# bioinfologics/w2rap-contigger

Measured on AMD Instinct MI355X. Metric: step2_k60_canonical_kmers_per_s, higher is better.
Workload: dtype u64

## Files before the change

### include/w2rap_step2.h

```cpp
#ifndef W2RAP_STEP2_H_
#define W2RAP_STEP2_H_

#include <stddef.h>
#include <stdint.h>

#ifdef __cplusplus
extern "C" {
#endif

#define W2RAP_STEP2_ABI_VERSION 3

enum {
    W2RAP_OK = 0,
    W2RAP_E_ARG = 1,
    W2RAP_E_NO_DEVICE = 2,
    W2RAP_E_HIP = 3,
    W2RAP_E_STATE = 4,
    W2RAP_E_LIMIT = 5,
    W2RAP_E_GRAPH = 6,
    W2RAP_E_HINT = 7,
    W2RAP_E_IO = 8
};

enum { W2RAP_MEM_HOST = 0, W2RAP_MEM_DEVICE = 1 };
// ... 3 lines not shown
    const uint8_t*  bases_packed;
    const uint64_t* base_byte_off;
    const uint32_t* read_len;
    const uint8_t*  quals;
    const uint64_t* qual_off;
    const uint8_t*  pq;
    const uint64_t* pq_off;
    int32_t mem;
} w2rap_reads;

typedef struct w2rap_edge_hint {
    uint64_t n_edges;
    const uint8_t*  packed;
    const uint64_t* byte_off;
    const uint32_t* len;
} w2rap_edge_hint;

typedef struct w2rap_step2_params {
    uint32_t K;
    uint32_t min_qual;
    uint32_t min_freq;
    int32_t  device;
    const w2rap_edge_hint* edge_order_hint;
    const char* freqs_path;
    int32_t  n_gpus;
    uint32_t n_passes;
    const int32_t* devices;
    uint32_t flags;
} w2rap_step2_params;
#define W2RAP_F_REPLICATED_GRAPH 1u
#define W2RAP_F_GRAPH_ONLY 2u

typedef struct w2rap_step2_out {
    int32_t  K;
    uint64_t n_vertices;
    uint64_t n_edge_objs;
    uint8_t*  edge_packed;
    uint64_t* edge_byte_off;
    uint32_t* edge_len;
    int32_t*  vleft;
    int32_t*  vright;
    uint64_t* from_off;
    int32_t*  from_v;
    int32_t*  from_e;
    uint64_t* to_off;
    int32_t*  to_v;
    int32_t*  to_e;
    uint64_t n_unipaths;
    int32_t*  fwd_xlat;
    int32_t*  rev_xlat;
    uint64_t n_paths;
    int32_t*  path_offset;
    uint64_t* path_off;
    int32_t*  path_edges;
    uint64_t hist[101];
    uint64_t n_kmer_instances;
    uint64_t n_kmers_distinct;
    uint64_t n_kmers_solid;
    uint64_t n_reads_pathed;
    uint64_t n_reads_multipathed;
    float ms_count, ms_graph, ms_path;
} w2rap_step2_out;

int  w2rap_step2_run(const w2rap_reads* reads, const w2rap_step2_params* params,
                     w2rap_step2_out* out, char* err, size_t errlen);
void w2rap_step2_free(w2rap_step2_out* out);
int  w2rap_step2_device_count(void);
int  w2rap_step2_abi_version(void);
int  w2rap_step2_last_peer_mode(void);

int  w2rap_step2_trim_cached(void);
struct w2rap_step2_ctx* w2rap_step2_acquire(int device, char* err, size_t errlen);
void w2rap_step2_release(struct w2rap_step2_ctx*);

typedef struct w2rap_step2_ctx w2rap_step2_ctx;

w2rap_step2_ctx* w2rap_step2_create(int device, char* err, size_t errlen);
void        w2rap_step2_destroy(w2rap_step2_ctx*);
const char* w2rap_step2_last_error(const w2rap_step2_ctx*);
int w2rap_step2_set_reads(w2rap_step2_ctx*, const w2rap_reads* reads);
int w2rap_step2_count_kmers(w2rap_step2_ctx*, uint32_t min_qual, uint32_t min_freq, w2rap_step2_out* stats);
int w2rap_step2_count_kmers_passes(w2rap_step2_ctx*, uint32_t min_qual, uint32_t min_freq, uint32_t n_passes, w2rap_step2_out* stats);
int w2rap_step2_build_graph(w2rap_step2_ctx*, const w2rap_edge_hint* hint);
int w2rap_step2_path_reads(w2rap_step2_ctx*);
int w2rap_step2_fetch(w2rap_step2_ctx*, w2rap_step2_out* out);
void* w2rap_step2_stream(w2rap_step2_ctx*);

int w2rap_step2_trim(w2rap_step2_ctx*);

int w2rap_step2_copy_bench(w2rap_step2_ctx*, uint64_t nbytes, uint32_t reps, double* gb_per_s);
int w2rap_step2_device_copy(w2rap_step2_ctx*, void* dst, const void* src, uint64_t nbytes);
int w2rap_step2_copy_bench_form(void);

int    w2rap_step2_set_profiling(w2rap_step2_ctx*, int on);
size_t w2rap_step2_profile(w2rap_step2_ctx*, char* buf, size_t len, int reset);

int w2rap_step2_counts(w2rap_step2_ctx*, uint64_t out[8]);

int w2rap_step2_get_good_len(w2rap_step2_ctx*, uint16_t* out );
int w2rap_step2_get_table(w2rap_step2_ctx*, uint64_t* hi, uint64_t* lo, uint8_t* count, uint8_t* ctx,
                          int32_t* edge, uint32_t* off );

int      w2rap_step2_quality_windows(w2rap_step2_ctx*, uint32_t min_qual, uint64_t* n_kmers );
uint32_t w2rap_step2_default_buckets(uint64_t total_kmers, uint32_t multiple_of);
uint32_t w2rap_step2_record_bytes(void);
int w2rap_step2_partition(w2rap_step2_ctx*, uint32_t n_buckets, uint32_t n_parts, uint64_t* recs_per_part,
                          uint64_t* kmers_per_part);
int w2rap_step2_partition_range(w2rap_step2_ctx*, uint32_t n_buckets, uint32_t first_bucket, uint32_t end_bucket, uint32_t n_parts,
                                uint64_t* recs_per_part, uint64_t* kmers_per_part);
int w2rap_step2_count_pass(w2rap_step2_ctx*, uint32_t pass, uint32_t n_passes);
int w2rap_step2_partition_buffers(w2rap_step2_ctx*, void** d_records, void** d_bucket_counts, uint64_t* n_records);
int w2rap_step2_count_records(w2rap_step2_ctx*, uint32_t min_freq, uint32_t n_local_buckets, uint32_t n_segments,
                              const void* d_records, const void* d_counts, uint64_t total_kmers, w2rap_step2_out* stats);
int w2rap_step2_count_records_begin(w2rap_step2_ctx*, uint32_t min_freq, uint32_t n_local_buckets, uint32_t n_segments,
                                    const void* d_records, const void* d_counts, uint64_t total_kmers, uint32_t n_slices,
                                    int deferred);
int w2rap_step2_count_records_slices(w2rap_step2_ctx*);
int w2rap_step2_count_records_bounds(w2rap_step2_ctx*, uint32_t k, uint32_t* first_bucket, uint32_t* end_bucket);
int w2rap_step2_count_records_launch(w2rap_step2_ctx*, uint32_t k);
int w2rap_step2_count_records_slice(w2rap_step2_ctx*, uint32_t k, uint64_t* n_solid, uint64_t* n_chunks);
int w2rap_step2_count_records_end(w2rap_step2_ctx*, w2rap_step2_out* stats);
int w2rap_step2_solid_buffers(w2rap_step2_ctx*, void** d_hi, void** d_lo, void** d_cc, uint64_t* n);
int w2rap_step2_set_solid(w2rap_step2_ctx*, const void* d_hi, const void* d_lo, const void* d_cc, uint64_t n,
                          uint64_t M, uint64_t D, const uint64_t* hist101);
int w2rap_step2_chunk_buffers(w2rap_step2_ctx*, void** d_chunk_start, void** d_chunk_count, uint64_t* n_chunks);
int w2rap_step2_set_solid_chunked(w2rap_step2_ctx*, const void* d_hi, const void* d_lo, const void* d_cc, uint64_t n,
                                  uint64_t M, uint64_t D, const uint64_t* hist101,
                                  const void* d_chunk_start, const void* d_chunk_count, uint64_t n_chunks);

int w2rap_step2_dict_begin(w2rap_step2_ctx*, uint64_t kmer_capacity, uint64_t chunk_capacity);
int w2rap_step2_dict_append(w2rap_step2_ctx*, const void* d_hi, const void* d_lo, const void* d_cc, uint64_t n,
                            const void* d_chunk_start, const void* d_chunk_count, uint64_t n_chunks);
int w2rap_step2_dict_append_slice(w2rap_step2_ctx*, const void* d_hi, const void* d_lo, const void* d_cc, uint64_t n,
                                  const void* d_chunk_start, const void* d_chunk_count, uint64_t n_chunks, uint64_t chunk_bias);
int w2rap_step2_dict_end(w2rap_step2_ctx*, uint64_t M, uint64_t D, const uint64_t* hist101);
int w2rap_step2_dict_abort(w2rap_step2_ctx*);

enum { W2RAP_X_DONE = 0, W2RAP_X_ALLTOALL = 1, W2RAP_X_ALLGATHER = 2, W2RAP_X_ALLGATHER_HOST = 3, W2RAP_X_ALLREDUCE_U8 = 4, W2RAP_X_ALLREDUCE_U32 = 5 };
typedef struct w2rap_xchg {
    int32_t  op;
    uint32_t elem_bytes;
    void*    send;
    uint64_t send_count[64];
} w2rap_xchg;
int w2rap_step2_shard_begin(w2rap_step2_ctx*, uint32_t rank, uint32_t world, const uint64_t* solid_per_rank ,
                            uint32_t n_buckets, uint32_t n_passes, uint64_t M, uint64_t D, const uint64_t* hist101,
                            const w2rap_edge_hint* hint );
int w2rap_step2_local_dict_slice(w2rap_step2_ctx*, uint64_t n_solid, uint64_t expected_total);
int w2rap_step2_shard_next(w2rap_step2_ctx*, w2rap_xchg* x);
int w2rap_step2_shard_recv(w2rap_step2_ctx*, const uint64_t* recv_count , uint32_t elem_bytes, void** d_recv);
int w2rap_step2_shard_host_words(w2rap_step2_ctx*, const uint64_t* words );
int w2rap_step2_shard_info(w2rap_step2_ctx*, uint64_t out[8]);
int w2rap_step2_selftest_prims(w2rap_step2_ctx*, uint64_t n, uint64_t seed, int key_bits);
uint64_t w2rap_step2_device_bytes(w2rap_step2_ctx*);
uint64_t w2rap_step2_device_peak_bytes(w2rap_step2_ctx*, int reset);

#ifdef __cplusplus
}
#endif
#endif
```

### w2rap_contigger_amd/csrc/step2_graph.hip

```cpp
#include <algorithm>
#include "ctx.h"

namespace w2 {

enum { GE_LOOKUP = 1, GE_OFFSET = 2, GE_HINT_MISS = 4, GE_HINT_DUP = 8, GE_ASSIGN = 16, GE_HINT_LEN = 32 };

template <class Id>
__device__ inline Kmer oriented(const uint64_t* shi, const uint64_t* slo, Id v) {
    Kmer k{shi[v >> 1], slo[v >> 1]};
    return (v & 1) ? kmer_rc(k) : k;
}

template <class Id>
__global__ void __launch_bounds__(256) k_links(uint64_t S, const uint64_t* __restrict__ shi, const uint64_t* __restrict__ slo,
                                                const uint8_t* __restrict__ sctx, Id* nbr_nxt0) {
    constexpr Id NONE = NodeId<Id>::NONE, PAL = NodeId<Id>::PAL;
    uint64_t i = (uint64_t)blockIdx.x * blockDim.x + threadIdx.x;
    if (i >= S) return;
    Kmer k{shi[i], slo[i]};
    Id n0 = NONE, n1 = NONE;
    if (!kmer_is_pal(k)) {
        const Id s = nbr_nxt0[2 * i], p = nbr_nxt0[2 * i + 1];
        if (s < PAL) {
            unsigned cj = sctx[s >> 1]; if (s & 1) cj = brev8(cj);
// ... 1203 lines not shown
    if (getenv("W2RAP_TRACE")) fprintf(stderr, "[w2rap] list ranking: %d jump launches\n", rounds);
    c.release(spl); c.release(d_cnt);
    if (mid) W2_HIP(hipMemsetAsync(mid, 0, N, st));
    LAUNCH(c, "k_rank_finish", k_rank_finish<Id>, dim3(grid_for(S)), dim3(256), 0, S, w, own, nxt0, shi, slo, nxt, rnk, cyc, mid, d_flags);
    W2_HIP(hipStreamSynchronize(st));
    return 0;
}
int run_ranking(Ctx& c, uint64_t N, const uint32_t* nxt0, uint32_t* nxt, uint32_t* rnk, unsigned long long* w, uint8_t* cyc, uint8_t* mid,
                uint32_t* d_flags, const uint64_t* shi, const uint64_t* slo, bool use_chunks) {
    uint32_t* own = nullptr;
    W2_ALLOC(own, uint32_t, N);
    const int rc = run_ranking_t<uint32_t>(c, N, nxt0, nxt, rnk, w, own, cyc, mid, d_flags, shi, slo, use_chunks);
    c.release(own);
    return rc;
}

static int graph_error(Ctx& c, uint32_t f) {
    if (f & GE_LOOKUP) { c.err = "neighbour k-mer lookup failed (ForceAssert, BuildReadQGraph.cc:265)"; return W2RAP_E_GRAPH; }
    if (f & GE_OFFSET) { c.err = "unipath longer than 16,777,215 k-mers (ForceAssertLe, ReadPather.h:122)"; return W2RAP_E_GRAPH; }
    if (f & GE_ASSIGN) { c.err = "k-mer left without an edge (BuildReadQGraph.cc:303)"; return W2RAP_E_GRAPH; }
    if (f & GE_HINT_MISS) { c.err = "edge_order_hint: a hinted edge is not a unipath of this graph"; return W2RAP_E_HINT; }
    if (f & GE_HINT_DUP) { c.err = "edge_order_hint: an edge is listed twice"; return W2RAP_E_HINT; }
    if (f & GE_HINT_LEN) { c.err = "edge_order_hint: a hinted edge has the wrong length"; return W2RAP_E_HINT; }
    return 0;
}

template <class Id>
static int rank_resolve_t(Ctx& c, uint64_t N, Id* nxt0, unsigned long long* rankw, uint32_t* own, uint8_t* cyc, uint8_t* mid, uint32_t* d_flags,
                          const uint64_t* shi, const uint64_t* slo, bool with_mid, bool* had_circles = nullptr) {
    hipStream_t st = c.stream;
    const uint64_t S = N / 2;
    uint32_t h_flags[4] = {0, 0, 0, 0};
    W2_TRY(run_ranking_t<Id>(c, N, nxt0, (Id*)nullptr, (uint32_t*)nullptr, rankw, own, cyc, mid, d_flags, with_mid ? shi : nullptr, slo, true));
    W2_HIP(hipMemcpyAsync(h_flags, d_flags, 16, hipMemcpyDeviceToHost, st));
    W2_HIP(hipStreamSynchronize(st));
    W2_TRY(graph_error(c, h_flags[1]));
    if (had_circles) *had_circles = h_flags[2] != 0;
    if (h_flags[2]) {
        Id *nx, *mn, *nx2, *mn2;
        W2_ALLOC(nx, Id, N); W2_ALLOC(mn, Id, N); W2_ALLOC(nx2, Id, N); W2_ALLOC(mn2, Id, N);
        LAUNCH(c, "k_minjump_init", k_minjump_init<Id>, dim3(grid_for(S)), dim3(256), 0, S, nxt0, cyc, nx, mn);
        for (int round = 0; round < 33; ++round) {
            LAUNCH(c, "k_minjump", k_minjump<Id>, dim3(grid_for(S)), dim3(256), 0, S, shi, slo, nx, mn, nx2, mn2);
            std::swap(nx, nx2); std::swap(mn, mn2);
        }
        LAUNCH(c, "k_cycle_cut", k_cycle_cut<Id>, dim3(grid_for(S)), dim3(256), 0, S, cyc, mn, nxt0);
        W2_HIP(hipStreamSynchronize(st));
        c.release(nx); c.release(mn); c.release(nx2); c.release(mn2);
        W2_HIP(hipMemsetAsync(d_flags, 0, 32, st));
        W2_TRY(run_ranking_t<Id>(c, N, nxt0, (Id*)nullptr, (uint32_t*)nullptr, rankw, own, cyc, mid, d_flags, with_mid ? shi : nullptr, slo, true));
        W2_HIP(hipMemcpyAsync(h_flags, d_flags, 16, hipMemcpyDeviceToHost, st));
        W2_HIP(hipStreamSynchronize(st));
        if (h_flags[2]) { c.err = "failed to close circle (BuildReadQGraph.cc:141)"; return W2RAP_E_GRAPH; }
    }
    return 0;
}
int rank_resolve32(Ctx& c, uint64_t N, uint32_t* nxt0, unsigned long long* rankw, uint32_t* own, uint8_t* cyc, uint8_t* mid, uint32_t* d_flags,
                   const uint64_t* shi, const uint64_t* slo, bool* had_circles) {
    return rank_resolve_t<uint32_t>(c, N, nxt0, rankw, own, cyc, mid, d_flags, shi, slo, false, had_circles);
}
int rank_resolve64(Ctx& c, uint64_t N, uint64_t* nxt0, unsigned long long* rankw, uint32_t* own, uint8_t* cyc, uint8_t* mid, uint32_t* d_flags,
                   const uint64_t* shi, const uint64_t* slo, bool* had_circles) {
    return rank_resolve_t<uint64_t>(c, N, nxt0, rankw, own, cyc, mid, d_flags, shi, slo, false, had_circles);
}

int graph_finish(Ctx& c) {
    hipStream_t st = c.stream;
    const uint64_t E = c.E;
    uint32_t* d_flags = nullptr;
    W2_ALLOC(d_flags, uint32_t, 8);
    W2_HIP(hipMemsetAsync(d_flags, 0, 32, st));
    uint32_t h_flags[4] = {0, 0, 0, 0};
    if (!c.bits_ready) {
        const uint64_t nby = (c.edge_bases + 3) / 4;
        W2_ALLOC(c.d_edge_bits, uint8_t, nby + 16);
        W2_HIP(hipMemsetAsync(c.d_edge_bits + nby, 0, 16, st));
        if (nby) LAUNCH(c, "k_pack_codes", k_pack_codes, dim3(grid_for(nby)), dim3(256), 0, nby, c.edge_bases, c.d_edge_codes, c.d_edge_bits);
    }
    c.bits_ready = false;
    if (c.use_index && c.d_table) { c.release(c.d_table); c.d_table = nullptr; }
    if (c.use_index && !c.index_prebuilt) W2_TRY(build_index(c));
    c.index_prebuilt = false;
    if (c.filter_prebuilt) c.filter_prebuilt = false;
    else {
    if (c.d_filter32) { c.release(c.d_filter32); c.d_filter32 = nullptr; }
    c.f32words = 0;
    if (c.edge_bases >= FMER && c.stream2 && !getenv("W2RAP_NO_FILTER32") && c.edge_bases <= (1ull << 33)) {
        uint64_t fw = 1024;
        while (fw * 4 < c.edge_bases) fw <<= 1;
        W2_ALLOC(c.d_filter32, unsigned long long, fw);
        c.f32words = fw;
        hipEvent_t ev;
        W2_HIP(hipEventCreateWithFlags(&ev, hipEventDisableTiming));
        W2_HIP(hipEventRecord(ev, st));
        W2_HIP(hipStreamWaitEvent(c.stream2, ev, 0));
        (void)hipEventDestroy(ev);
        W2_HIP(hipMemsetAsync(c.d_filter32, 0, fw * 8, c.stream2));
        const uint64_t npos = c.edge_bases - (FMER - 1);
        LAUNCH_ON(c, c.stream2, "k_filter32", k_filter32, dim3(grid_for(npos)), dim3(256), 0, npos, c.d_edge_bits, c.d_filter32, (uint32_t)(fw - 1), 0u, (uint32_t)fw);
    }
    }
    uint32_t* d_nobj = nullptr; uint64_t* d_ooff = nullptr;
    W2_ALLOC(d_nobj, uint32_t, E); W2_ALLOC(d_ooff, uint64_t, E + 1);
    if (E) LAUNCH(c, "k_edge_nobj", k_edge_nobj, dim3(grid_for(E)), dim3(256), 0, E, c.d_edge_nk, c.d_edge_off, c.d_edge_codes, d_nobj);
    W2_TRY(exclusive_scan_u32_to_u64(c, d_nobj, d_ooff, E));
    W2_HIP(hipMemcpyAsync(&c.NO, d_ooff + E, 8, hipMemcpyDeviceToHost, st));
    W2_HIP(hipMemcpyAsync(h_flags, d_flags, 16, hipMemcpyDeviceToHost, st));
    W2_HIP(hipStreamSynchronize(st));
    W2_TRY(graph_error(c, h_flags[1]));
    const uint64_t NO = c.NO;
    if (NO >= (1ull << 31)) { c.err = "more than 2^31 edge objects"; return W2RAP_E_LIMIT; }
    W2_ALLOC(c.d_fwdX, int32_t, E); W2_ALLOC(c.d_revX, int32_t, E); W2_ALLOC(c.d_obj_edge, uint32_t, NO);
    W2_ALLOC(c.d_left, int32_t, NO); W2_ALLOC(c.d_right, int32_t, NO);
    if (E) LAUNCH(c, "k_edge_xlat", k_edge_xlat, dim3(grid_for(E)), dim3(256), 0, E, d_nobj, d_ooff, c.d_fwdX, c.d_revX, c.d_obj_edge);
    const uint64_t NE = 2 * NO;
    uint64_t *ehash, *ehi, *elo, *ktmp, *excl;
    uint32_t *eperm, *eflag;
    W2_ALLOC(ehash, uint64_t, NE); W2_ALLOC(ehi, uint64_t, NE); W2_ALLOC(elo, uint64_t, NE); W2_ALLOC(ktmp, uint64_t, NE);
    W2_ALLOC(excl, uint64_t, NE + 1); W2_ALLOC(eperm, uint32_t, NE); W2_ALLOC(eflag, uint32_t, NE);
    c.NV = 0;
    if (NE) {
        LAUNCH(c, "k_ends", k_ends, dim3(grid_for(NE)), dim3(256), 0, NO, c.d_obj_edge, c.d_edge_off, c.d_edge_nk, c.d_edge_codes, ehash, ehi, elo);
        bool by_bases = test_hook("W2RAP_TEST_ENDS_FULL_SORT");
        uint64_t nflag = 0;
        for (;;) {
            LAUNCH(c, "k_iota", k_iota, dim3(grid_for(NE)), dim3(256), 0, NE, eperm);
            if (by_bases) {
                LAUNCH(c, "k_gather_u64", k_gather_u64, dim3(grid_for(NE)), dim3(256), 0, NE, elo, eperm, ktmp);
                W2_TRY(sort_pairs_u64(c, ktmp, eperm, NE, 0, 58));
                LAUNCH(c, "k_gather_u64", k_gather_u64, dim3(grid_for(NE)), dim3(256), 0, NE, ehi, eperm, ktmp);
                W2_TRY(sort_pairs_u64(c, ktmp, eperm, NE, 0, 60));
            }
            LAUNCH(c, "k_gather_u64", k_gather_u64, dim3(grid_for(NE)), dim3(256), 0, NE, ehash, eperm, ktmp);
            W2_TRY(sort_pairs_u64(c, ktmp, eperm, NE, 0, 64));
            W2_HIP(hipMemsetAsync(d_flags + 3, 0, 4, st));
            LAUNCH(c, "k_end_flags", k_end_flags, dim3(grid_for(NE)), dim3(256), 0, NE, eperm, ehash, ehi, elo, eflag, d_flags + 3);
            W2_TRY(exclusive_scan_u32_to_u64(c, eflag, excl, NE));
            uint32_t shared_hash = 0;
            W2_HIP(hipMemcpyAsync(&nflag, excl + NE, 8, hipMemcpyDeviceToHost, st));
            W2_HIP(hipMemcpyAsync(&shared_hash, d_flags + 3, 4, hipMemcpyDeviceToHost, st));
            W2_HIP(hipStreamSynchronize(st));
            if (shared_hash && !by_bases) { by_bases = true; continue; }
            break;
        }
        c.NV = nflag + 1;
        LAUNCH(c, "k_end_vertices", k_end_vertices, dim3(grid_for(NE)), dim3(256), 0, NE, eperm, eflag, excl, c.d_left, c.d_right);
    }
    const uint64_t NV = c.NV;
    W2_ALLOC(c.d_from_off, uint64_t, NV + 1); W2_ALLOC(c.d_to_off, uint64_t, NV + 1);
    W2_ALLOC(c.d_from_v, int32_t, NO); W2_ALLOC(c.d_from_e, int32_t, NO);
    W2_ALLOC(c.d_to_v, int32_t, NO); W2_ALLOC(c.d_to_e, int32_t, NO);
    uint32_t* deg = nullptr; uint64_t* akeys = nullptr; uint32_t* avals = nullptr;
    W2_ALLOC(deg, uint32_t, NV); W2_ALLOC(akeys, uint64_t, NO); W2_ALLOC(avals, uint32_t, NO);
    for (int dir = 0; dir < 2; ++dir) {
        const int32_t* a = dir == 0 ? c.d_left : c.d_right;
        const int32_t* b = dir == 0 ? c.d_right : c.d_left;
        W2_HIP(hipMemsetAsync(deg, 0, (NV ? NV : 1) * 4, st));
        if (NO) {
            LAUNCH(c, "k_adj_keys", k_adj_keys, dim3(grid_for(NO)), dim3(256), 0, NO, a, b, akeys, avals, deg);
            W2_TRY(sort_pairs_u64(c, akeys, avals, NO, 0, 64));
            LAUNCH(c, "k_adj_out", k_adj_out, dim3(grid_for(NO)), dim3(256), 0, NO, avals, b, dir == 0 ? c.d_from_v : c.d_to_v,
                               dir == 0 ? c.d_from_e : c.d_to_e);
        }
        W2_TRY(exclusive_scan_u32_to_u64(c, deg, dir == 0 ? c.d_from_off : c.d_to_off, NV));
    }
    if (c.d_otab) { c.release(c.d_otab); c.d_otab = nullptr; }
    W2_ALLOC(c.d_otab, ObjRec, NO);
    if (NO) LAUNCH(c, "k_obj_table", k_obj_table, dim3(grid_for(NO)), dim3(256), 0, NO, c.d_obj_edge, c.d_edge_nk, c.d_edge_off, c.d_edge_codes,
                   c.d_right, c.d_from_off, c.d_from_e, c.d_otab);
    W2_HIP(hipStreamSynchronize(st));
    if (c.stream2) W2_HIP(hipStreamSynchronize(c.stream2));
    W2_HIP(hipGetLastError());
    for (void* p : {(void*)d_nobj, (void*)d_ooff, (void*)ehash, (void*)ehi, (void*)elo, (void*)ktmp, (void*)excl,
                    (void*)eperm, (void*)eflag, (void*)deg, (void*)akeys, (void*)avals, (void*)d_flags})
        c.release(p);
    c.graphed = true;
    return 0;
}

template <class Id>
static int phase_graph_t(Ctx& c, const w2rap_edge_hint* hint) {
    constexpr Id NONE = NodeId<Id>::NONE; (void)NONE;
    hipStream_t st = c.stream;
    const uint64_t S = c.S, N = 2 * S;
    const uint64_t mask = c.tcap - 1;
    uint32_t* d_flags = nullptr;
    W2_ALLOC(d_flags, uint32_t, 8);
    W2_HIP(hipMemsetAsync(d_flags, 0, 32, st));
    Id* nxt0 = reinterpret_cast<Id*>(c.d_nbr);
    unsigned long long* rankw = nullptr; uint32_t* own = nullptr;
    W2_ALLOC(rankw, unsigned long long, N); W2_ALLOC(own, uint32_t, N);
    uint8_t *cyc = nullptr, *mid = nullptr, *is_head = nullptr;
    W2_ALLOC(cyc, uint8_t, N); W2_ALLOC(mid, uint8_t, N);
    uint32_t h_flags[4] = {0, 0, 0, 0};
    if (S) {
        LAUNCH(c, "k_links", k_links<Id>, dim3(grid_for(S)), dim3(256), 0, S, c.d_shi, c.d_slo, c.d_sctx, nxt0);
        W2_TRY(rank_resolve_t<Id>(c, N, nxt0, rankw, own, cyc, mid, d_flags, c.d_shi, c.d_slo, true));
    }
    c.release(cyc); cyc = nullptr;
    unsigned long long* d_nheads = nullptr;
    W2_ALLOC(d_nheads, unsigned long long, 1);
    W2_HIP(hipMemsetAsync(d_nheads, 0, 8, st));
    const uint64_t head_cap = S ? c.rank_ends + 1 : 1;
    Id *head_v, *edge_head; uint32_t* perm;
    uint64_t *key_hi, *key_lo, *key_tmp;
    W2_ALLOC(is_head, uint8_t, N);
    W2_ALLOC(head_v, Id, head_cap); W2_ALLOC(key_hi, uint64_t, head_cap); W2_ALLOC(key_lo, uint64_t, head_cap);
    if (S) LAUNCH(c, "k_heads", k_heads<Id>, dim3((unsigned)((S + 256 * HEADS_PER - 1) / (256 * HEADS_PER))), dim3(256), 0, S, c.d_shi, c.d_slo, nxt0, own, rankw, mid, is_head,
                              head_v, key_hi, key_lo, d_nheads, head_cap, d_flags, hint == nullptr);
    W2_HIP(hipGetLastError());
    unsigned long long E = 0;
    W2_HIP(hipMemcpyAsync(&E, d_nheads, 8, hipMemcpyDeviceToHost, st));
    W2_HIP(hipMemcpyAsync(h_flags, d_flags, 16, hipMemcpyDeviceToHost, st));
    W2_HIP(hipStreamSynchronize(st));
    W2_TRY(graph_error(c, h_flags[1]));
    if (E > head_cap) { c.err = "more canonical heads than chain ends"; return W2RAP_E_GRAPH; }
    if (E >= (1ull << 31)) { c.err = "more than 2^31 unipaths (edge ids are int, paths/long/ReadPath.h)"; return W2RAP_E_LIMIT; }
    c.E = E;
    c.release(c.d_nbr); c.d_nbr = nullptr; nxt0 = nullptr;
    c.release(mid); mid = nullptr;
    W2_ALLOC(perm, uint32_t, E); W2_ALLOC(edge_head, Id, E);
    W2_ALLOC(key_tmp, uint64_t, E);
    W2_ALLOC(c.d_edge_nk, uint32_t, E);
    if (hint) {
        if (hint->n_edges != E) {
            c.err = "edge_order_hint has " + std::to_string(hint->n_edges) + " edges, the graph has " + std::to_string(E);
            return W2RAP_E_HINT;
        }
        std::vector<uint64_t> hh(E), hl(E);
        for (uint64_t e = 0; e < E; ++e) {
            if (hint->len[e] < K) { c.err = "edge_order_hint: edge shorter than K"; return W2RAP_E_HINT; }
            const uint8_t* p = hint->packed + hint->byte_off[e];
            uint64_t hi = 0, lo = 0;
            for (unsigned t = 0; t < 30; ++t) hi = (hi << 2) | ((p[t >> 2] >> (2 * (t & 3))) & 3);
            for (unsigned t = 30; t < 60; ++t) lo = (lo << 2) | ((p[t >> 2] >> (2 * (t & 3))) & 3);
            hh[e] = hi; hl[e] = lo;
        }
        uint32_t* d_hlen = nullptr;
        W2_ALLOC(d_hlen, uint32_t, E);
        W2_HIP(hipMemcpyAsync(key_hi, hh.data(), E * 8, hipMemcpyHostToDevice, st));
        W2_HIP(hipMemcpyAsync(key_lo, hl.data(), E * 8, hipMemcpyHostToDevice, st));
        W2_HIP(hipMemcpyAsync(d_hlen, hint->len, E * 4, hipMemcpyHostToDevice, st));
        if (E) LAUNCH(c, "k_edge_from_hint", k_edge_from_hint<Id>, dim3(grid_for(E)), dim3(256), 0, E, key_hi, key_lo, d_hlen, c.d_table, mask, c.d_shi, c.d_slo, is_head,
                                  own, rankw, edge_head, c.d_edge_nk, d_flags);
        W2_HIP(hipMemcpyAsync(h_flags, d_flags, 16, hipMemcpyDeviceToHost, st));
        W2_HIP(hipStreamSynchronize(st));
        W2_TRY(graph_error(c, h_flags[1]));
        c.release(d_hlen);
    } else {
        if (E) {
            unsigned max_run = 64;
            if (test_hook("W2RAP_TEST_TIE_RUN")) max_run = (unsigned)atoi(getenv("W2RAP_TEST_TIE_RUN"));
            LAUNCH(c, "k_iota", k_iota, dim3(grid_for(E)), dim3(256), 0, E, perm);
            W2_HIP(hipMemcpyAsync(key_tmp, key_hi, E * 8, hipMemcpyDeviceToDevice, st));
            W2_TRY(sort_pairs_u64(c, key_tmp, perm, E, 0, 60));
            W2_HIP(hipMemsetAsync(d_flags + 3, 0, 4, st));
            LAUNCH(c, "k_tie_sort_lo", k_tie_sort_lo, dim3(grid_for(E)), dim3(256), 0, E, key_tmp, key_lo, perm, max_run, d_flags + 3);
            uint32_t long_run = 0;
            W2_HIP(hipMemcpyAsync(&long_run, d_flags + 3, 4, hipMemcpyDeviceToHost, st));
            W2_HIP(hipStreamSynchronize(st));
            if (long_run) {
                LAUNCH(c, "k_iota", k_iota, dim3(grid_for(E)), dim3(256), 0, E, perm);
                W2_TRY(sort_pairs_u64(c, key_lo, perm, E, 0, 60));
                LAUNCH(c, "k_gather_u64", k_gather_u64, dim3(grid_for(E)), dim3(256), 0, E, key_hi, perm, key_tmp);
                W2_TRY(sort_pairs_u64(c, key_tmp, perm, E, 0, 60));
            }
            LAUNCH(c, "k_edge_from_sorted", k_edge_from_sorted<Id>, dim3(grid_for(E)), dim3(256), 0, E, perm, head_v, own, rankw, edge_head, c.d_edge_nk);
        }
    }
    W2_HIP(hipStreamSynchronize(st));
    c.release(is_head); is_head = nullptr;
    uint32_t* d_elen = nullptr;
    W2_ALLOC(d_elen, uint32_t, E);
    W2_ALLOC(c.d_edge_off, uint64_t, E + 1);
    if (E) LAUNCH(c, "k_edge_len", k_edge_len, dim3(grid_for(E)), dim3(256), 0, E, c.d_edge_nk, d_elen);
    W2_TRY(exclusive_scan_u32_to_u64(c, d_elen, c.d_edge_off, E));
    W2_HIP(hipMemcpyAsync(&c.edge_bases, c.d_edge_off + E, 8, hipMemcpyDeviceToHost, st));
    W2_HIP(hipStreamSynchronize(st));
    W2_ALLOC(c.d_edge_codes, uint8_t, c.edge_bases + 64);
    {
        const char* iv = getenv("W2RAP_PATH_INDEX");
        c.use_index = iv && atoi(iv) != 0;
    }
    if (c.d_srec) { c.release(c.d_srec); c.d_srec = nullptr; }
    if (!c.use_index) W2_ALLOC(c.d_srec, KRec, S);
    if (S) LAUNCH(c, "k_assign", k_assign<Id>, dim3(grid_for(S)), dim3(256), 0, S, c.d_shi, c.d_slo, own, rankw,
                              c.d_edge_off, c.d_srec, c.d_edge_codes, d_flags);
    W2_HIP(hipStreamSynchronize(st));
    c.release(rankw); c.release(own); rankw = nullptr; own = nullptr;
    for (void* p : {(void*)d_nheads, (void*)head_v, (void*)perm, (void*)edge_head, (void*)key_hi, (void*)key_lo, (void*)key_tmp, (void*)d_elen, (void*)d_flags})
        c.release(p);
    return graph_finish(c);
}

int phase_graph(Ctx& c, const w2rap_edge_hint* hint) {
    if (!c.counted) { c.err = "build_graph called before count_kmers"; return W2RAP_E_STATE; }
    if (!c.d_nbr && c.S) { c.err = "build_graph: the neighbour links of this count have been consumed; call count_kmers again"; return W2RAP_E_STATE; }
    c.graphed = false;
    return c.wide_ids ? phase_graph_t<uint64_t>(c, hint) : phase_graph_t<uint32_t>(c, hint);
}

}
```

### w2rap_contigger_amd/csrc/step2_prims.hip

```cpp
#include <algorithm>
#include <cstring>
#include <vector>
#include <rocprim/rocprim.hpp>
#include "ctx.h"

namespace w2 {

static void* tmp_alloc(Ctx& c, size_t bytes) { return c.alloc<uint8_t>(bytes ? bytes : 16, false); }

constexpr unsigned SCAN_THREADS = 256, SCAN_ITEMS = 16, SCAN_TILE = SCAN_THREADS * SCAN_ITEMS;
constexpr unsigned long long ST_EMPTY = 0, ST_AGG = 1ull << 62, ST_PREFIX = 2ull << 62, ST_VAL = (1ull << 62) - 1;

struct OpPlus { __device__ static inline uint64_t id() { return 0; } __device__ static inline uint64_t f(uint64_t a, uint64_t b) { return a + b; } };
struct OpMax { __device__ static inline uint64_t id() { return 0; } __device__ static inline uint64_t f(uint64_t a, uint64_t b) { return a > b ? a : b; } };

__device__ inline bool load16_u32(const uint32_t* q, uint32_t (&t)[16]) {
    if ((uintptr_t)q & 15) return false;
    const uint4* q4 = reinterpret_cast<const uint4*>(q);
#pragma unroll
    for (unsigned k = 0; k < 4; ++k) { const uint4 w = q4[k]; t[4 * k] = w.x; t[4 * k + 1] = w.y; t[4 * k + 2] = w.z; t[4 * k + 3] = w.w; }
    return true;
}
struct InU32 {
    const uint32_t* p;
// ... 144 lines not shown
int inclusive_max_scan_u32(Ctx& c, const uint32_t* in, uint32_t* out, uint64_t n) { return run_scan<InU32, OpMax, uint32_t, false>(c, InU32{in}, out, n, c.stream); }

__global__ void __launch_bounds__(256) k_max_u32(const uint32_t* __restrict__ in, uint64_t n, uint32_t* __restrict__ out) {
    uint32_t m = 0;
    for (uint64_t i = (uint64_t)blockIdx.x * blockDim.x + threadIdx.x; i < n; i += (uint64_t)gridDim.x * blockDim.x) m = max(m, in[i]);
    for (int d = 32; d > 0; d >>= 1) m = max(m, (uint32_t)__shfl_down((int)m, d));
    if ((threadIdx.x & 63) == 0 && m) atomicMax(out, m);
}
int max_u32(Ctx& c, const uint32_t* in, uint64_t n, uint32_t* result) {
    *result = 0;
    if (!n) return 0;
    uint32_t* d_out = c.alloc<uint32_t>(1, false);
    if (!d_out) return W2RAP_E_HIP;
    W2_HIP(hipMemsetAsync(d_out, 0, 4, c.stream));
    const unsigned grid = (unsigned)std::min<uint64_t>((n + 255) / 256, (uint64_t)c.sm_count * 8);
    hipLaunchKernelGGL(k_max_u32, dim3(grid), dim3(256), 0, c.stream, in, n, d_out);
    W2_HIP(hipMemcpyAsync(result, d_out, sizeof(uint32_t), hipMemcpyDeviceToHost, c.stream));
    W2_HIP(hipStreamSynchronize(c.stream));
    c.release(d_out);
    return 0;
}

constexpr unsigned RS_THREADS = 256, RS_ITEMS = 8, RS_TILE = RS_THREADS * RS_ITEMS, RS_BITS = 8, RS_DIGITS = 1u << RS_BITS, RS_MAXPASS = 8;
static_assert(RS_DIGITS == RS_THREADS, "thread = digit in the look-back");
__global__ void __launch_bounds__(RS_THREADS) k_rs_totals(const uint64_t* __restrict__ keys, uint64_t n, int begin_bit, int end_bit, unsigned long long* __restrict__ tot) {
    __shared__ uint32_t s_h[RS_MAXPASS][RS_DIGITS];
    const unsigned tid = threadIdx.x;
    for (unsigned p = 0; p < RS_MAXPASS; ++p) s_h[p][tid] = 0;
    __syncthreads();
    for (uint64_t i = (uint64_t)blockIdx.x * blockDim.x + tid; i < n; i += (uint64_t)gridDim.x * blockDim.x) {
        const uint64_t k = keys[i];
        unsigned p = 0;
        for (int sh = begin_bit; sh < end_bit; sh += RS_BITS, ++p) atomicAdd(&s_h[p][(k >> sh) & ((1u << min(RS_BITS, (unsigned)(end_bit - sh))) - 1u)], 1u);
    }
    __syncthreads();
    for (unsigned p = 0; p < RS_MAXPASS; ++p) if (s_h[p][tid]) atomicAdd(&tot[p * RS_DIGITS + tid], (unsigned long long)s_h[p][tid]);
}
__global__ void __launch_bounds__(RS_THREADS) k_rs_onesweep(const uint64_t* __restrict__ keys, const uint32_t* __restrict__ vals, uint64_t n, unsigned shift, unsigned dmask,
                                                             const unsigned long long* __restrict__ tot ,
                                                             unsigned long long* __restrict__ status , unsigned long long* __restrict__ ticket,
                                                             uint64_t* __restrict__ kout, uint32_t* __restrict__ vout) {
    __shared__ uint32_t s_run[RS_DIGITS];
    __shared__ uint32_t s_cnt[RS_THREADS / 64][RS_DIGITS];
    __shared__ unsigned long long s_base[RS_DIGITS];
    __shared__ unsigned long long s_scan[RS_THREADS / 64];
    __shared__ unsigned long long s_tile;
    const unsigned tid = threadIdx.x, lane = tid & 63, wv = tid >> 6;
    if (tid == 0) s_tile = atomicAdd(ticket, 1ull);
    s_run[tid] = 0;
    __syncthreads();
    const uint64_t blk = s_tile, base = blk * RS_TILE;
    uint64_t key[RS_ITEMS]; uint32_t rank[RS_ITEMS];
#pragma unroll
    for (unsigned j = 0; j < RS_ITEMS; ++j) {
#pragma unroll
        for (unsigned w = 0; w < RS_THREADS / 64; ++w) s_cnt[w][tid] = 0;
        __syncthreads();
        const uint64_t i = base + (uint64_t)j * RS_THREADS + tid;
        const bool live = i < n;
        key[j] = live ? keys[i] : 0;
        const unsigned d = (unsigned)(key[j] >> shift) & dmask;
        unsigned long long peers = __ballot(live);
#pragma unroll
        for (unsigned b = 0; b < RS_BITS; ++b) {
            const unsigned long long m = __ballot((d >> b) & 1u);
            peers &= ((d >> b) & 1u) ? m : ~m;
        }
        const unsigned before = (unsigned)__builtin_popcountll(peers & ((1ull << lane) - 1));
        if (live && before == 0) s_cnt[wv][d] = (unsigned)__builtin_popcountll(peers);
        __syncthreads();
        unsigned off = s_run[d];
        for (unsigned w = 0; w < wv; ++w) off += s_cnt[w][d];
        rank[j] = off + before;
        __syncthreads();
        {
            uint32_t add = 0;
#pragma unroll
            for (unsigned w = 0; w < RS_THREADS / 64; ++w) add += s_cnt[w][tid];
            s_run[tid] += add;
        }
        __syncthreads();
    }
    {
        const unsigned long long t = tot[tid];
        unsigned long long incl = t;
#pragma unroll
        for (int dd = 1; dd < 64; dd <<= 1) { const unsigned long long o = __shfl_up(incl, dd); if ((int)lane >= dd) incl += o; }
        if (lane == 63) s_scan[wv] = incl;
        __syncthreads();
        unsigned long long wbase = 0;
        for (unsigned w = 0; w < wv; ++w) wbase += s_scan[w];
        const unsigned long long below = wbase + incl - t;
        const unsigned long long mine = s_run[tid];
        unsigned long long* st = status + blk * RS_DIGITS;
        unsigned long long excl = 0;
        if (blk == 0) __hip_atomic_store(&st[tid], ST_PREFIX | mine, __ATOMIC_RELAXED, __HIP_MEMORY_SCOPE_AGENT);
        else {
            __hip_atomic_store(&st[tid], ST_AGG | mine, __ATOMIC_RELAXED, __HIP_MEMORY_SCOPE_AGENT);
            for (uint64_t p = blk; p-- > 0;) {
                unsigned long long sv;
                do { sv = __hip_atomic_load(&status[p * RS_DIGITS + tid], __ATOMIC_RELAXED, __HIP_MEMORY_SCOPE_AGENT); } while ((sv >> 62) == 0);
                excl += sv & ST_VAL;
                if ((sv >> 62) == 2) break;
            }
            __hip_atomic_store(&st[tid], ST_PREFIX | (excl + mine), __ATOMIC_RELAXED, __HIP_MEMORY_SCOPE_AGENT);
        }
        s_base[tid] = below + excl;
    }
    __syncthreads();
#pragma unroll
    for (unsigned j = 0; j < RS_ITEMS; ++j) {
        const uint64_t i = base + (uint64_t)j * RS_THREADS + tid;
        if (i < n) {
            const unsigned d = (unsigned)(key[j] >> shift) & dmask;
            const unsigned long long pos = s_base[d] + rank[j];
            kout[pos] = key[j]; vout[pos] = vals[i];
        }
    }
}

int own_sort_pairs(Ctx& c, uint64_t* keys, uint32_t* vals, uint64_t n, int begin_bit, int end_bit) {
    hipStream_t st = c.stream;
    if (end_bit - begin_bit > (int)(RS_BITS * RS_MAXPASS)) { c.err = "sort: more than 64 key bits"; return W2RAP_E_ARG; }
    const unsigned nblocks = (unsigned)((n + RS_TILE - 1) / RS_TILE);
    const unsigned npass = (unsigned)((end_bit - begin_bit + RS_BITS - 1) / RS_BITS);
    uint64_t* k2 = c.alloc<uint64_t>(n, false);
    uint32_t* v2 = c.alloc<uint32_t>(n, false);
    const uint64_t nstat = (uint64_t)nblocks * RS_DIGITS + 1;
    unsigned long long* work = c.alloc<unsigned long long>(RS_MAXPASS * RS_DIGITS + npass * nstat, false);
    if (!k2 || !v2 || !work) return W2RAP_E_HIP;
    unsigned long long* tot = work; unsigned long long* stat = work + RS_MAXPASS * RS_DIGITS;
    W2_HIP(hipMemsetAsync(work, 0, (RS_MAXPASS * RS_DIGITS + npass * nstat) * 8, st));
    uint64_t *ka = keys, *kb = k2; uint32_t *va = vals, *vb = v2;
    c.pbegin("k_radix_sort_pairs");
    hipLaunchKernelGGL(k_rs_totals, dim3(std::min<unsigned>(nblocks, (unsigned)c.sm_count * 4)), dim3(RS_THREADS), 0, st, (const uint64_t*)keys, n, begin_bit, end_bit, tot);
    unsigned p = 0;
    for (int shift = begin_bit; shift < end_bit; shift += RS_BITS, ++p) {
        const unsigned dmask = (1u << std::min<int>(RS_BITS, end_bit - shift)) - 1u;
        hipLaunchKernelGGL(k_rs_onesweep, dim3(nblocks), dim3(RS_THREADS), 0, st, (const uint64_t*)ka, (const uint32_t*)va, n, (unsigned)shift, dmask,
                           (const unsigned long long*)(tot + p * RS_DIGITS), stat + p * nstat, stat + p * nstat + (nstat - 1), kb, vb);
        std::swap(ka, kb); std::swap(va, vb);
    }
    if (ka != keys) {
        W2_HIP(hipMemcpyAsync(keys, ka, n * sizeof(uint64_t), hipMemcpyDeviceToDevice, st));
        W2_HIP(hipMemcpyAsync(vals, va, n * sizeof(uint32_t), hipMemcpyDeviceToDevice, st));
    }
    c.pend();
    W2_HIP(hipGetLastError());
    W2_HIP(hipStreamSynchronize(st));
    c.release(k2); c.release(v2); c.release(work);
    return 0;
}

int sort_pairs_u64(Ctx& c, uint64_t* keys, uint32_t* vals, uint64_t n, int begin_bit, int end_bit) {
    if (n < 2 || end_bit <= begin_bit) return 0;
    if (n <= (1ull << 24) && !getenv("W2RAP_ROCPRIM_SORT")) return own_sort_pairs(c, keys, vals, n, begin_bit, end_bit);
    uint64_t* k2 = c.alloc<uint64_t>(n, false);
    uint32_t* v2 = c.alloc<uint32_t>(n, false);
    if (!k2 || !v2) return W2RAP_E_HIP;
    size_t tmp_bytes = 0;
    W2_HIP(rocprim::radix_sort_pairs(nullptr, tmp_bytes, keys, k2, vals, v2, n, begin_bit, end_bit, c.stream));
    void* tmp = tmp_alloc(c, tmp_bytes);
    if (!tmp) return W2RAP_E_HIP;
    c.pbegin("rocprim_radix_sort_pairs");
    W2_HIP(rocprim::radix_sort_pairs(tmp, tmp_bytes, keys, k2, vals, v2, n, begin_bit, end_bit, c.stream));
    W2_HIP(hipMemcpyAsync(keys, k2, n * sizeof(uint64_t), hipMemcpyDeviceToDevice, c.stream));
    W2_HIP(hipMemcpyAsync(vals, v2, n * sizeof(uint32_t), hipMemcpyDeviceToDevice, c.stream));
    c.pend();
    W2_HIP(hipStreamSynchronize(c.stream));
    c.release(tmp); c.release(k2); c.release(v2);
    return 0;
}

}

extern "C" int w2rap_step2_selftest_prims(w2rap_step2_ctx* h, uint64_t n, uint64_t seed, int key_bits) {
    if (!h) return -1;
    w2::Ctx& c = h->c;
    if (hipSetDevice(c.device) != hipSuccess) return -1;
    std::vector<uint64_t> hk(n); std::vector<uint32_t> hv(n), hu(n);
    uint64_t x = seed * 0x9E3779B97F4A7C15ull + 1;
    for (uint64_t i = 0; i < n; ++i) {
        x ^= x << 13; x ^= x >> 7; x ^= x << 17;
        hk[i] = (key_bits >= 64 || key_bits < 0) ? x : (x & ((1ull << key_bits) - 1));
        if (i % 5 == 0 && i) hk[i] = hk[i - 1];
        hv[i] = (uint32_t)i;
        hu[i] = (uint32_t)(x >> 40) & 1023u;
    }
    uint64_t *dk = c.alloc<uint64_t>(n + 1, false), *dk2 = c.alloc<uint64_t>(n + 1, false), *ds = c.alloc<uint64_t>(n + 2, false);
    uint32_t *dv = c.alloc<uint32_t>(n + 1, false), *dv2 = c.alloc<uint32_t>(n + 1, false), *du = c.alloc<uint32_t>(n + 1, false), *dm = c.alloc<uint32_t>(n + 1, false);
    if (!dk || !dk2 || !ds || !dv || !dv2 || !du || !dm) return -1;
    auto up = [&](void* d, const void* s, size_t b) { return b ? hipMemcpy(d, s, b, hipMemcpyHostToDevice) : hipSuccess; };
    auto dn = [&](void* d, const void* s, size_t b) { return b ? hipMemcpy(d, s, b, hipMemcpyDeviceToHost) : hipSuccess; };
    int bad = 0;
    if (up(dk, hk.data(), n * 8) != hipSuccess || up(dv, hv.data(), n * 4) != hipSuccess || up(dk2, hk.data(), n * 8) != hipSuccess || up(dv2, hv.data(), n * 4) != hipSuccess ||
        up(du, hu.data(), n * 4) != hipSuccess) return -1;
    const int eb = key_bits < 0 ? -key_bits : key_bits >= 64 ? 64 : key_bits;
    const uint64_t smask = eb >= 64 ? ~0ull : ((1ull << eb) - 1);
    if (n >= 2) {
        if (w2::own_sort_pairs(c, dk, dv, n, 0, eb)) return -1;
        std::vector<uint32_t> perm(n);
        for (uint64_t i = 0; i < n; ++i) perm[i] = (uint32_t)i;
        std::stable_sort(perm.begin(), perm.end(), [&](uint32_t a, uint32_t b) { return (hk[a] & smask) < (hk[b] & smask); });
        std::vector<uint64_t> gk(n); std::vector<uint32_t> gv(n);
        if (dn(gk.data(), dk, n * 8) != hipSuccess || dn(gv.data(), dv, n * 4) != hipSuccess) return -1;
        for (uint64_t i = 0; i < n && !bad; ++i) { if (gk[i] != hk[perm[i]]) bad = 1; else if (gv[i] != perm[i]) bad = 2; }
    }
    if (!bad) {
        if (w2::exclusive_scan_u32_to_u64(c, du, ds, n)) return -1;
        std::vector<uint64_t> gs(n + 1);
        if (dn(gs.data(), ds, (n + 1) * 8) != hipSuccess) return -1;
        uint64_t run = 0;
        for (uint64_t i = 0; i < n && !bad; ++i) { if (gs[i] != run) bad = 3; run += hu[i]; }
        if (!bad && gs[n] != run) bad = 4;
    }
    if (!bad && n) {
        if (w2::inclusive_max_scan_u32(c, du, dm, n)) return -1;
        std::vector<uint32_t> gm(n);
        if (dn(gm.data(), dm, n * 4) != hipSuccess) return -1;
        uint32_t mx = 0;
        for (uint64_t i = 0; i < n && !bad; ++i) { mx = std::max(mx, hu[i]); if (gm[i] != mx) bad = 5; }
        uint32_t r = 0;
        if (w2::max_u32(c, du, n, &r)) return -1;
        if (!bad && r != mx) bad = 6;
    }
    if (!bad) {
        if (w2::exclusive_scan_u64(c, dk2, ds, n)) return -1;
        std::vector<uint64_t> gs(n + 1);
        if (dn(gs.data(), ds, (n + 1) * 8) != hipSuccess) return -1;
        uint64_t run = 0;
        if (key_bits > 0 && key_bits <= 40) for (uint64_t i = 0; i <= n && !bad; ++i) { if (gs[i] != run) bad = 7; if (i < n) run += hk[i]; }
    }
    if (!bad) {
        std::vector<uint32_t> a(n);
        for (uint64_t i = 0; i < n; ++i) a[i] = (hu[i] & 3) ? (uint32_t)i : (uint32_t)(i / 2);
        if (up(dv2, a.data(), n * 4) != hipSuccess) return -1;
        if (w2::exclusive_scan_is_self(c, dv2, ds, n)) return -1;
        std::vector<uint64_t> gs(n + 1);
        if (dn(gs.data(), ds, (n + 1) * 8) != hipSuccess) return -1;
        uint64_t run = 0;
        for (uint64_t i = 0; i <= n && !bad; ++i) { if (gs[i] != run) bad = 8; if (i < n) run += a[i] == (uint32_t)i; }
    }
    for (void* p : {(void*)dk, (void*)dk2, (void*)ds, (void*)dv, (void*)dv2, (void*)du, (void*)dm}) c.release(p);
    return bad;
}
```

Measured before the change: 40.87 billion.

## Add small-input MSD radix sort path and narrow adjacency sort key bits

```diff
diff --git a/include/w2rap_step2.h b/include/w2rap_step2.h
--- a/include/w2rap_step2.h
+++ b/include/w2rap_step2.h
@@ -179,6 +179,8 @@
 int w2rap_step2_shard_host_words(w2rap_step2_ctx*, const uint64_t* words );
 int w2rap_step2_shard_info(w2rap_step2_ctx*, uint64_t out[8]);
 int w2rap_step2_selftest_prims(w2rap_step2_ctx*, uint64_t n, uint64_t seed, int key_bits);
+int w2rap_step2_test_sort_pairs(w2rap_step2_ctx*, uint64_t* keys, uint32_t* vals, uint64_t n, int begin_bit, int end_bit, int route, int* taken,
+                                float* ms);
 uint64_t w2rap_step2_device_bytes(w2rap_step2_ctx*);
 uint64_t w2rap_step2_device_peak_bytes(w2rap_step2_ctx*, int reset);
 
diff --git a/w2rap_contigger_amd/csrc/step2_graph.hip b/w2rap_contigger_amd/csrc/step2_graph.hip
--- a/w2rap_contigger_amd/csrc/step2_graph.hip
+++ b/w2rap_contigger_amd/csrc/step2_graph.hip
@@ -1379,13 +1379,14 @@
     W2_ALLOC(c.d_to_v, int32_t, NO); W2_ALLOC(c.d_to_e, int32_t, NO);
     uint32_t* deg = nullptr; uint64_t* akeys = nullptr; uint32_t* avals = nullptr;
     W2_ALLOC(deg, uint32_t, NV); W2_ALLOC(akeys, uint64_t, NO); W2_ALLOC(avals, uint32_t, NO);
+    const int adj_bits = 32 + (NV > 1 ? 64 - __builtin_clzll(NV - 1) : 0);
     for (int dir = 0; dir < 2; ++dir) {
         const int32_t* a = dir == 0 ? c.d_left : c.d_right;
         const int32_t* b = dir == 0 ? c.d_right : c.d_left;
         W2_HIP(hipMemsetAsync(deg, 0, (NV ? NV : 1) * 4, st));
         if (NO) {
             LAUNCH(c, "k_adj_keys", k_adj_keys, dim3(grid_for(NO)), dim3(256), 0, NO, a, b, akeys, avals, deg);
-            W2_TRY(sort_pairs_u64(c, akeys, avals, NO, 0, 64));
+            W2_TRY(sort_pairs_u64(c, akeys, avals, NO, 0, adj_bits));
             LAUNCH(c, "k_adj_out", k_adj_out, dim3(grid_for(NO)), dim3(256), 0, NO, avals, b, dir == 0 ? c.d_from_v : c.d_to_v,
                                dir == 0 ? c.d_from_e : c.d_to_e);
         }
diff --git a/w2rap_contigger_amd/csrc/step2_prims.hip b/w2rap_contigger_amd/csrc/step2_prims.hip
--- a/w2rap_contigger_amd/csrc/step2_prims.hip
+++ b/w2rap_contigger_amd/csrc/step2_prims.hip
@@ -320,8 +320,183 @@
     return 0;
 }
 
+constexpr unsigned SS_THREADS = 256, SS_ITEMS = 16, SS_TILE = SS_THREADS * SS_ITEMS, SS_CAP = 5120;
+constexpr uint64_t SS_MAX_N = 1ull << 20;
+static_assert(SS_THREADS == 256 && RS_BITS == 8, "thread = digit");
+
+__device__ inline unsigned ss_round_rank(unsigned d, bool live, uint32_t (*s_cnt)[SS_THREADS], uint32_t* s_run) {
+    const unsigned tid = threadIdx.x, lane = tid & 63, wv = tid >> 6;
+#pragma unroll
+    for (unsigned w = 0; w < SS_THREADS / 64; ++w) s_cnt[w][tid] = 0;
+    __syncthreads();
+    unsigned long long peers = __ballot(live);
+#pragma unroll
+    for (unsigned b = 0; b < RS_BITS; ++b) {
+        const unsigned long long m = __ballot((d >> b) & 1u);
+        peers &= ((d >> b) & 1u) ? m : ~m;
+    }
+    const unsigned before = (unsigned)__builtin_popcountll(peers & ((1ull << lane) - 1));
+    if (live && before == 0) s_cnt[wv][d] = (unsigned)__builtin_popcountll(peers);
+    __syncthreads();
+    unsigned off = s_run[d];
+    for (unsigned w = 0; w < wv; ++w) off += s_cnt[w][d];
+    __syncthreads();
+    uint32_t add = 0;
+#pragma unroll
+    for (unsigned w = 0; w < SS_THREADS / 64; ++w) add += s_cnt[w][tid];
+    s_run[tid] += add;
+    __syncthreads();
+    return off + before;
+}
+__device__ inline uint64_t ss_block_excl(uint64_t v, unsigned long long* s_scan , uint64_t* total) {
+    const unsigned tid = threadIdx.x, lane = tid & 63, wv = tid >> 6;
+    uint64_t incl = v;
+#pragma unroll
+    for (int dd = 1; dd < 64; dd <<= 1) { const uint64_t o = __shfl_up(incl, dd); if ((int)lane >= dd) incl += o; }
+    if (lane == 63) s_scan[wv] = incl;
+    __syncthreads();
+    uint64_t wbase = 0, all = 0;
+#pragma unroll
+    for (unsigned w = 0; w < SS_THREADS / 64; ++w) { if (w < wv) wbase += s_scan[w]; all += s_scan[w]; }
+    __syncthreads();
+    *total = all;
+    return wbase + incl - v;
+}
+__global__ void __launch_bounds__(SS_THREADS) k_ss_count(const uint64_t* __restrict__ keys, uint64_t n, unsigned shift, unsigned dmask, uint32_t* __restrict__ cnt) {
+    __shared__ uint32_t s_h[RS_DIGITS];
+    const unsigned tid = threadIdx.x;
+    s_h[tid] = 0;
+    __syncthreads();
+    const uint64_t base = (uint64_t)blockIdx.x * SS_TILE;
+#pragma unroll
+    for (unsigned j = 0; j < SS_ITEMS; ++j) {
+        const uint64_t i = base + (uint64_t)j * SS_THREADS + tid;
+        if (i < n) atomicAdd(&s_h[(unsigned)(keys[i] >> shift) & dmask], 1u);
+    }
+    __syncthreads();
+    cnt[(uint64_t)blockIdx.x * RS_DIGITS + tid] = s_h[tid];
+}
+__global__ void __launch_bounds__(SS_THREADS) k_ss_scatter(const uint64_t* __restrict__ keys, const uint32_t* __restrict__ vals, uint64_t n, unsigned shift, unsigned dmask,
+                                                            const uint32_t* __restrict__ cnt, unsigned ntiles, uint64_t cap, uint64_t* __restrict__ kout, uint32_t* __restrict__ vout,
+                                                            uint64_t* __restrict__ bstart , uint32_t* __restrict__ over) {
+    __shared__ uint32_t s_run[RS_DIGITS];
+    __shared__ uint32_t s_cnt[SS_THREADS / 64][SS_THREADS];
+    __shared__ uint64_t s_base[RS_DIGITS];
+    __shared__ unsigned long long s_scan[SS_THREADS / 64];
+    const unsigned tid = threadIdx.x, blk = blockIdx.x;
+    {
+        uint64_t all = 0, before = 0;
+        for (unsigned t = 0; t < ntiles; ++t) { const uint32_t x = cnt[(uint64_t)t * RS_DIGITS + tid]; all += x; if (t < blk) before += x; }
+        uint64_t tot = 0;
+        const uint64_t below = ss_block_excl(all, s_scan, &tot);
+        s_base[tid] = below + before;
+        s_run[tid] = 0;
+        const int big = __syncthreads_or(all > cap), one = __syncthreads_or(all == n);
+        if (blk == 0) {
+            bstart[tid] = below;
+            if (tid == 0) { bstart[RS_DIGITS] = tot; *over = big ? (one ? 2u : 1u) : 0u; }
+        }
+    }
+    const uint64_t base = (uint64_t)blk * SS_TILE;
+    for (unsigned j = 0; j < SS_ITEMS; ++j) {
+        const uint64_t i = base + (uint64_t)j * SS_THREADS + tid;
+        const bool live = i < n;
+        const uint64_t k = live ? keys[i] : 0;
+        const unsigned d = (unsigned)(k >> shift) & dmask;
+        const unsigned r = ss_round_rank(d, live, s_cnt, s_run);
+        if (live) { const uint64_t pos = s_base[d] + r; kout[pos] = k; vout[pos] = vals[i]; }
+    }
+}
+__global__ void __launch_bounds__(SS_THREADS) k_ss_finish(const uint64_t* __restrict__ kin, const uint32_t* __restrict__ vin, const uint64_t* __restrict__ bstart,
+                                                           uint64_t kmask, unsigned shift2, unsigned dmask2, uint64_t* __restrict__ keys, uint32_t* __restrict__ vals) {
+    __shared__ uint64_t s_k[SS_CAP];
+    __shared__ uint16_t s_i[SS_CAP];
+    __shared__ uint32_t s_run[RS_DIGITS];
+    __shared__ uint32_t s_cnt[SS_THREADS / 64][SS_THREADS];
+    __shared__ uint32_t s_sub[RS_DIGITS + 1];
+    __shared__ unsigned long long s_scan[SS_THREADS / 64];
+    const unsigned tid = threadIdx.x;
+    const uint64_t s = bstart[blockIdx.x], L = bstart[blockIdx.x + 1] - s;
+    if (L == 0) return;
+    if (L > SS_CAP || dmask2 == 0) {
+        for (uint64_t i = tid; i < L; i += SS_THREADS) { keys[s + i] = kin[s + i]; vals[s + i] = vin[s + i]; }
+        return;
+    }
+    const unsigned n = (unsigned)L;
+    s_run[tid] = 0;
+    __syncthreads();
+    for (unsigned i = tid; i < n; i += SS_THREADS) atomicAdd(&s_run[(unsigned)(kin[s + i] >> shift2) & dmask2], 1u);
+    __syncthreads();
+    {
+        uint64_t tot = 0;
+        const uint32_t h = s_run[tid];
+        s_sub[tid] = (uint32_t)ss_block_excl(h, s_scan, &tot);
+        if (tid == 0) s_sub[RS_DIGITS] = n;
+        s_run[tid] = 0;
+    }
+    __syncthreads();
+    for (unsigned r0 = 0; r0 < n; r0 += SS_THREADS) {
+        const unsigned i = r0 + tid;
+        const bool live = i < n;
+        const uint64_t k = live ? kin[s + i] : 0;
+        const unsigned d = (unsigned)(k >> shift2) & dmask2;
+        const unsigned r = ss_round_rank(d, live, s_cnt, s_run);
+        if (live) { const unsigned p = s_sub[d] + r; s_k[p] = k; s_i[p] = (uint16_t)i; }
+    }
+    __syncthreads();
+    for (unsigned p = tid; p < n; p += SS_THREADS) {
+        const uint64_t k = s_k[p], km = k & kmask;
+        const unsigned d = (unsigned)(k >> shift2) & dmask2;
+        const unsigned lo = s_sub[d], hi = s_sub[d + 1];
+        unsigned r = lo;
+        for (unsigned j = lo; j < hi; ++j) {
+            const uint64_t kj = s_k[j] & kmask;
+            r += (kj < km || (kj == km && j < p)) ? 1u : 0u;
+        }
+        keys[s + r] = k; vals[s + r] = vin[s + s_i[p]];
+    }
+}
+
+static int small_sort_pairs(Ctx& c, uint64_t* keys, uint32_t* vals, uint64_t n, int begin_bit, int end_bit, int* route) {
+    hipStream_t st = c.stream;
+    const uint64_t ntiles64 = (n + SS_TILE - 1) / SS_TILE;
+    if (ntiles64 >= (1ull << 31)) { c.err = "sort: too many elements"; return W2RAP_E_LIMIT; }
+    const unsigned ntiles = (unsigned)ntiles64;
+    const int shift = std::max(begin_bit, end_bit - (int)RS_BITS), shift2 = std::max(begin_bit, shift - (int)RS_BITS);
+    const unsigned dmask = (1u << (end_bit - shift)) - 1u, dmask2 = shift > shift2 ? (1u << (shift - shift2)) - 1u : 0u;
+    const int span = end_bit - begin_bit;
+    const uint64_t kmask = (span >= 64 ? ~0ull : ((1ull << span) - 1)) << begin_bit;
+    uint64_t* k2 = c.alloc<uint64_t>(n, false);
+    uint32_t* v2 = c.alloc<uint32_t>(n, false);
+    uint64_t* bstart = c.alloc<uint64_t>(RS_DIGITS + 2, false);
+    uint32_t* cnt = c.alloc<uint32_t>((uint64_t)ntiles * RS_DIGITS, false);
+    if (!k2 || !v2 || !bstart || !cnt) return W2RAP_E_HIP;
+    uint32_t* over = (uint32_t*)(bstart + RS_DIGITS + 1);
+    c.pbegin("k_radix_sort_small");
+    hipLaunchKernelGGL(k_ss_count, dim3(ntiles), dim3(SS_THREADS), 0, st, (const uint64_t*)keys, n, (unsigned)shift, dmask, cnt);
+    hipLaunchKernelGGL(k_ss_scatter, dim3(ntiles), dim3(SS_THREADS), 0, st, (const uint64_t*)keys, (const uint32_t*)vals, n, (unsigned)shift, dmask,
+                       (const uint32_t*)cnt, ntiles, shift > begin_bit ? (uint64_t)SS_CAP : ~0ull, k2, v2, bstart, over);
+    hipLaunchKernelGGL(k_ss_finish, dim3(dmask + 1), dim3(SS_THREADS), 0, st, (const uint64_t*)k2, (const uint32_t*)v2, (const uint64_t*)bstart, kmask,
+                       (unsigned)shift2, dmask2, keys, vals);
+    c.pend();
+    uint32_t h_over = 0;
+    W2_HIP(hipMemcpyAsync(&h_over, over, 4, hipMemcpyDeviceToHost, st));
+    W2_HIP(hipGetLastError());
+    W2_HIP(hipStreamSynchronize(st));
+    c.release(k2); c.release(v2); c.release(bstart); c.release(cnt);
+    if (h_over == 2) return small_sort_pairs(c, keys, vals, n, begin_bit, shift, route);
+    *route = h_over ? 2 : 1;
+    return h_over ? own_sort_pairs(c, keys, vals, n, begin_bit, end_bit) : 0;
+}
+
+static bool small_sort_enabled() { const char* e = getenv("W2RAP_SORT_SMALL"); return !(e && e[0] == '0'); }
+
 int sort_pairs_u64(Ctx& c, uint64_t* keys, uint32_t* vals, uint64_t n, int begin_bit, int end_bit) {
     if (n < 2 || end_bit <= begin_bit) return 0;
+    if (n <= SS_MAX_N && end_bit - begin_bit > (int)RS_BITS && end_bit - begin_bit <= 64 && small_sort_enabled() && !getenv("W2RAP_ROCPRIM_SORT")) {
+        int route = 0;
+        return small_sort_pairs(c, keys, vals, n, begin_bit, end_bit, &route);
+    }
     if (n <= (1ull << 24) && !getenv("W2RAP_ROCPRIM_SORT")) return own_sort_pairs(c, keys, vals, n, begin_bit, end_bit);
     uint64_t* k2 = c.alloc<uint64_t>(n, false);
     uint32_t* v2 = c.alloc<uint32_t>(n, false);
@@ -412,3 +587,28 @@
     for (void* p : {(void*)dk, (void*)dk2, (void*)ds, (void*)dv, (void*)dv2, (void*)du, (void*)dm}) c.release(p);
     return bad;
 }
+
+extern "C" int w2rap_step2_test_sort_pairs(w2rap_step2_ctx* h, uint64_t* keys, uint32_t* vals, uint64_t n, int begin_bit, int end_bit, int route,
+                                           int* taken, float* ms) {
+    if (!h || !keys || !vals || !taken || !ms || begin_bit < 0 || end_bit > 64 || begin_bit >= end_bit) return -1;
+    w2::Ctx& c = h->c;
+    if (hipSetDevice(c.device) != hipSuccess) return -1;
+    *taken = 0; *ms = 0;
+    if (n < 2) return 0;
+    uint64_t* dk = c.alloc<uint64_t>(n, false);
+    uint32_t* dv = c.alloc<uint32_t>(n, false);
+    if (!dk || !dv) return -1;
+    if (hipMemcpy(dk, keys, n * 8, hipMemcpyHostToDevice) != hipSuccess || hipMemcpy(dv, vals, n * 4, hipMemcpyHostToDevice) != hipSuccess) return -1;
+    int rc;
+    {
+        w2::Timer t(c.stream);
+        rc = route == 1 ? w2::small_sort_pairs(c, dk, dv, n, begin_bit, end_bit, taken)
+           : route == 2 ? w2::own_sort_pairs(c, dk, dv, n, begin_bit, end_bit)
+                        : w2::sort_pairs_u64(c, dk, dv, n, begin_bit, end_bit);
+        *ms = t.stop();
+    }
+    if (route == 0 && !rc && n <= w2::SS_MAX_N && end_bit - begin_bit > (int)w2::RS_BITS && w2::small_sort_enabled() && !getenv("W2RAP_ROCPRIM_SORT")) *taken = -1;
+    if (rc || hipMemcpy(keys, dk, n * 8, hipMemcpyDeviceToHost) != hipSuccess || hipMemcpy(vals, dv, n * 4, hipMemcpyDeviceToHost) != hipSuccess) return -1;
+    c.release(dk); c.release(dv);
+    return 0;
+}
```

Result: no change. 40.82 billion (median of 4 runs) (-0.1%).
